# VinAIResearch/GeoFormer

Hardware: AMD Instinct MI355X
Metric: scenes/sec forward (ScanNetV2 ~150k pts) (higher is better)
Workload: dtype f32

## Files before the change

### geoformer_amd/csrc/host_draw.hip

```cpp
#include <stdint.h>
#include <stdlib.h>
#include <string.h>

#include "common.h"

#if defined(__x86_64__) && !defined(__HIP_DEVICE_COMPILE__)
#include <immintrin.h>
#define GF_DRAW_AVX2 1
#endif

namespace {
constexpr int MT_N = 624, MT_M = 397;

__attribute__((always_inline)) inline void mt_advance_body(uint32_t* key) {
    constexpr uint32_t A = 0x9908b0dfu, UP = 0x80000000u, LO = 0x7fffffffu;
    int i = 0;
    for (; i < MT_N - MT_M; i++) {
        const uint32_t y = (key[i] & UP) | (key[i + 1] & LO);
        key[i] = key[i + MT_M] ^ (y >> 1) ^ ((0u - (y & 1u)) & A);
    }
    for (; i < MT_N - 1; i++) {
        const uint32_t y = (key[i] & UP) | (key[i + 1] & LO);
        key[i] = key[i + (MT_M - MT_N)] ^ (y >> 1) ^ ((0u - (y & 1u)) & A);
    }
// ... 257 lines not shown
    }
    if (out)
        for (long long t = 0; t < k; t++) out[t] = (long long)x[t];
    if (out32 && (uint32_t*)out32 != x) memcpy(out32, x, (size_t)k * sizeof(int32_t));
    *pos_io = pos;
    return GF_OK;
}

__global__ void k_take_drawn(const int32_t* __restrict__ idx, int k, int n, const float* __restrict__ xyz_src,
                             long long* __restrict__ idx64, float* __restrict__ xyz_dst, int32_t* __restrict__ idx32) {
    const int t = blockIdx.x * blockDim.x + threadIdx.x;
    if (t >= k) return;
    const int j = idx[t];
    idx64[t] = j;
    idx32[t] = j;
    if ((unsigned)j >= (unsigned)n) return;
    xyz_dst[3 * t + 0] = xyz_src[3 * (size_t)j + 0];
    xyz_dst[3 * t + 1] = xyz_src[3 * (size_t)j + 1];
    xyz_dst[3 * t + 2] = xyz_src[3 * (size_t)j + 2];
}

extern "C" int gf_host_draw_sample(uint32_t* key, int32_t* pos_io, long long n, long long k, int32_t* pinned,
                                   long long pinned_cap, int32_t* d_idx32, long long* d_idx64, const float* xyz_src,
                                   float* xyz_dst, int fps_m, int32_t* fps_idx, void* fps_scratch, void* stream) {
    GF_CHECK_ARG(key && pos_io && pinned && d_idx32 && d_idx64 && xyz_src && xyz_dst, "gf_host_draw_sample: null argument");
    GF_CHECK_ARG(n >= 1 && n <= 0x7fffffffLL && k >= 1 && k <= n && pinned_cap >= k, "gf_host_draw_sample: n=%lld k=%lld cap=%lld",
                 n, k, pinned_cap);
    GF_CHECK_ARG(*pos_io >= 0 && *pos_io <= MT_N, "gf_host_draw_sample: generator position %d", (int)*pos_io);
    const int rc = legacy_choice32(key, pos_io, n, k, pinned, pinned_cap);
    if (rc != GF_OK) return rc;
    hipStream_t st = (hipStream_t)stream;
    hipLaunchKernelGGL(k_take_drawn, dim3((unsigned)gf_div_up(k, 256)), dim3(256), 0, st, pinned, (int)k, (int)n, xyz_src, d_idx64,
                       xyz_dst, d_idx32);
    GF_CHECK_LAUNCH("gf_host_draw_sample");
    if (fps_m > 0) {
        GF_CHECK_ARG(fps_idx && fps_scratch, "gf_host_draw_sample: sampling outputs missing");
        return gf_furthest_point_sampling(xyz_dst, 1, (int)k, fps_m, fps_idx, fps_scratch, stream);
    }
    return GF_OK;
}
```

### geoformer_amd/csrc/pointops.hip

```cpp
#include <stdlib.h>

#include <type_traits>

#include "common.h"

__global__ void k_voxelize_fp(const float* __restrict__ feats, const int32_t* __restrict__ rules, int M, int maxActive,
                              int C, int average, float* __restrict__ out) {
    long long t = (long long)blockIdx.x * blockDim.x + threadIdx.x;
    if (t >= (long long)M * C) return;
    const int row = (int)(t / C), c = (int)(t - (long long)row * C);
    const int32_t* r = rules + (size_t)row * (maxActive + 1);
    const int n = r[0];
    const float mult = (average && n > 0) ? __fdiv_rn(1.0f, (float)n) : 1.0f;
    float acc = 0.f;
    for (int i = 1; i <= n; i++) acc = __fadd_rn(acc, __fmul_rn(mult, feats[(size_t)r[i] * C + c]));
    out[t] = acc;
}

__global__ void k_voxelize_bp(const float* __restrict__ d_out, const int32_t* __restrict__ rules, int M, int maxActive,
                              int C, int average, float* __restrict__ d_feats) {
    long long t = (long long)blockIdx.x * blockDim.x + threadIdx.x;
    if (t >= (long long)M * C) return;
    const int row = (int)(t / C), c = (int)(t - (long long)row * C);
    const int32_t* r = rules + (size_t)row * (maxActive + 1);
// ... 249 lines not shown
    if (__popcll(owners) == 1) {
        key = (unsigned)__builtin_amdgcn_readlane((int)key, __builtin_ctzll(owners));
    } else {
        const unsigned cand = dbits == md ? (FPS_KEY_NONE - key) : 0u;
        key = FPS_KEY_NONE - wave_max_u32(cand);
    }
    dbits = md;
}

template <int I, int N, typename F>
__device__ __forceinline__ void fps_static_for(F&& f) {
    if constexpr (I < N) {
        f(std::integral_constant<int, I>{});
        fps_static_for<I + 1, N>(f);
    }
}

#ifndef FPS_WAVES
#define FPS_WAVES 16
#endif
#ifndef FPS_MAXG
#define FPS_MAXG 16
#endif
#ifndef FPS_KPUB
#define FPS_KPUB 4
#endif
#ifndef FPS_K
#define FPS_K 16
#endif
#define FPS_PW (FPS_WAVES - FPS_WAVES / 4)
#ifndef FPS_POLL_SLEEP
#define FPS_POLL_SLEEP 4
#endif
#define FPS_NG (FPS_MAXG * FPS_KPUB / 64)
#define FPS_TAG (1ull << 63)

__device__ __forceinline__ unsigned long long fps_code(unsigned dbits, unsigned key) {
    return ((unsigned long long)dbits << 32) | ((unsigned long long)(FPS_KEY_NONE - key) << 1);
}
__device__ __forceinline__ unsigned long long wave_max_u64(unsigned long long c) {
    const unsigned hi = (unsigned)(c >> 32), md = wave_max_u32(hi);
    const unsigned long long owners = __ballot(hi == md);
    unsigned ml;
    if (__popcll(owners) == 1) {
        ml = (unsigned)__builtin_amdgcn_readlane((int)(unsigned)c, __builtin_ctzll(owners));
    } else {
        ml = wave_max_u32(hi == md ? (unsigned)c : 0u);
    }
    return ((unsigned long long)md << 32) | ml;
}
__device__ __forceinline__ int fps_code_index(unsigned long long c) {
    return c ? (int)((FPS_KEY_NONE - (unsigned)((c >> 1) & 0x7fffffffull)) & 0x3fffffu) : 0;
}

#ifdef FPS_TRACE
__device__ unsigned long long* g_fps_trace = nullptr;
extern "C" int gf_dev_fps_trace(void* p) {
// ... 4 lines not shown
#define FTA(i, a, b) do { ftr[i] += (b) - (a); } while (0)
#else
#define FT() 0ull
#define FTA(i, a, b) do { } while (0)
#endif

#define FPS_LDS_ST(p, v) __hip_atomic_store((p), (v), __ATOMIC_RELAXED, __HIP_MEMORY_SCOPE_WORKGROUP)
#define FPS_LDS_LD(p) __hip_atomic_load((p), __ATOMIC_RELAXED, __HIP_MEMORY_SCOPE_WORKGROUP)
#define FPS_ORDER() asm volatile("" ::: "memory")
template <int P>
__device__ __forceinline__ void fps_absorb(const float (&px)[P], const float (&py)[P], const float (&pz)[P], float (&tmp)[P],
                                           float ax, float ay, float az) {
#pragma unroll
    for (int i = 0; i < P; i++) {
        const float dx = px[i] - ax, dy = py[i] - ay, dz = pz[i] - az;
        tmp[i] = fminf(fmaf(dz, dz, fmaf(dy, dy, dx * dx)), tmp[i]);
    }
}

template <int P>
__global__ __launch_bounds__(FPS_WAVES * 64) void k_fps(const float* __restrict__ xyz, int n, int m, int m0, int G,
                                                        int bs_log2, int batch0,
                                                        unsigned long long* __restrict__ slots,
                                                        int32_t* __restrict__ idxs, int* __restrict__ err) {
    static_assert(FPS_NG >= 1 && FPS_NG * 64 == FPS_MAXG * FPS_KPUB && FPS_KPUB <= FPS_K && FPS_WAVES * 2 <= 64,
                  "lane mappings of the exchange");
    __shared__ unsigned long long s_part[2][FPS_WAVES * 2];
    __shared__ float s_xyz[2][FPS_K * 3];
    __shared__ unsigned s_prog[2];
    const int bi = batch0 + blockIdx.y, wg = blockIdx.x;
    xyz += (size_t)bi * n * 3;
    idxs += (size_t)bi * m;
    slots += (size_t)bi * 2 * FPS_MAXG * FPS_KPUB;
    const int lane = threadIdx.x & 63, wid = threadIdx.x >> 6;
    const bool holder = (wid & 3) != 0;
    const int hid = wid - 1 - (wid >> 2);
    const int gtid = (wg * FPS_PW + hid) * 64 + lane;
    const int stride = G * FPS_PW * 64;
    if (threadIdx.x < 2) s_prog[threadIdx.x] = 0u;
    if (!holder && lane < 4) s_part[lane >> 1][wid * 2 + (lane & 1)] = 0ull;

    float px[P], py[P], pz[P], tmp[P];
    unsigned key[P];
    unsigned elig = 0;
    const unsigned bs_mask = (1u << bs_log2) - 1u;
#pragma unroll
    for (int i = 0; i < P; i++) {
        const int k = gtid + i * stride;
        px[i] = py[i] = pz[i] = 0.f;
        tmp[i] = 1e10f;
        key[i] = FPS_KEY_NONE;
        if (holder && k < n) {
            px[i] = xyz[(size_t)k * 3 + 0];
            py[i] = xyz[(size_t)k * 3 + 1];
            pz[i] = xyz[(size_t)k * 3 + 2];
            const float mag = fmaf(pz[i], pz[i], fmaf(py[i], py[i], px[i] * px[i]));
            if (!((double)mag <= 1e-3)) elig |= 1u << i;
            const unsigned rev = bs_log2 ? (__brev((unsigned)k & bs_mask) >> (32 - bs_log2)) : 0u;
            key[i] = (rev << 22) | (unsigned)k;
        }
    }
    if (m0 <= 0 && wg == 0 && threadIdx.x == 0) idxs[0] = 0;
    int nnew = 1;
    float nx[FPS_K], ny[FPS_K], nz[FPS_K];
    nx[0] = xyz[0]; ny[0] = xyz[1]; nz[0] = xyz[2];
#pragma unroll
    for (int a = 1; a < FPS_K; a++) nx[a] = ny[a] = nz[a] = 0.f;
    int done = 1;
    if (m0 > 1) {
        for (int base = 0; base < m0 - 1; base += FPS_K) {
            const int cntk = min(FPS_K, m0 - 1 - base);
#pragma unroll
            for (int a = 0; a < FPS_K; a++) {
                const int pi = a < cntk ? idxs[base + a] : 0;
                nx[a] = xyz[(size_t)pi * 3 + 0];
                ny[a] = xyz[(size_t)pi * 3 + 1];
                nz[a] = xyz[(size_t)pi * 3 + 2];
            }
#pragma unroll
            for (int i = 0; i < P; i++) {
                if (elig & (1u << i)) {
                    float d2 = tmp[i];
#pragma unroll
                    for (int a = 0; a < FPS_K; a++) {
                        if (a < cntk) {
                            const float dx = px[i] - nx[a], dy = py[i] - ny[a], dz = pz[i] - nz[a];
                            d2 = fminf(fmaf(dz, dz, fmaf(dy, dy, dx * dx)), d2);
                        }
                    }
                    tmp[i] = d2;
                }
            }
        }
        const int pl = idxs[m0 - 1];
        nx[0] = xyz[(size_t)pl * 3 + 0];
        ny[0] = xyz[(size_t)pl * 3 + 1];
        nz[0] = xyz[(size_t)pl * 3 + 2];
        done = m0;
    }
#ifdef FPS_TRACE
    unsigned long long ftr[10] = {0, 0, 0, 0, 0, 0, 0, 0, 0, 0};
#endif
    if (holder) {
#pragma unroll
        for (int i = 0; i < P; i++) {
            if (elig & (1u << i)) {
                const float dx = px[i] - nx[0], dy = py[i] - ny[0], dz = pz[i] - nz[0];
// ... 2 lines not shown
        }
    } else {
        __builtin_amdgcn_s_setprio(3);
    }
    __syncthreads();
    for (int round = 1; done < m; round++) {
        const int par = round & 1;
        const unsigned long long ft0 = FT();
        unsigned bd = 0u, bk = FPS_KEY_NONE;
#pragma unroll
        for (int i = 0; i < P; i++) {
            if (elig & (1u << i)) {
                float d2 = tmp[i];
                const unsigned db = __float_as_uint(d2);
                if (db > bd || (db == bd && key[i] < bk)) {
                    bd = db;
                    bk = key[i];
                }
            }
        }
        const unsigned long long ft1 = FT();
        FTA(0, ft0, ft1);
        if (holder) {
        unsigned d1 = bd, k1 = bk;
        wave_best(d1, k1);
        unsigned cd = bd, ck = bk;
        if (bk == k1 && k1 != FPS_KEY_NONE) {
            cd = 0u;
            ck = FPS_KEY_NONE;
#pragma unroll
            for (int i = 0; i < P; i++) {
                if ((elig & (1u << i)) && key[i] != k1) {
                    const unsigned db = __float_as_uint(tmp[i]);
                    if (db > cd || (db == cd && key[i] < ck)) {
                        cd = db;
                        ck = key[i];
                    }
                }
            }
        }
        unsigned d2w = cd, k2w = ck;
        wave_best(d2w, k2w);
        if (lane == 0) {
            unsigned long long c1 = fps_code(d1, k1), c2 = fps_code(d2w, k2w);
            if (c2 != 0ull) c2 |= 1ull;
            else if (c1 != 0ull) c1 |= 1ull;
            s_part[par][wid * 2 + 0] = c1;
            s_part[par][wid * 2 + 1] = c2;
        }
        }
        const unsigned long long ft2 = FT();
        FTA(1, ft1, ft2);
        __syncthreads();
        const unsigned long long ft3 = FT();
        FTA(2, ft2, ft3);
        if (wid == 0) {
            unsigned long long mine = lane < FPS_WAVES * 2 ? s_part[par][lane] : 0ull;
            unsigned long long wgc[FPS_KPUB];
            bool stop = false;
            int cnt = 0;
            fps_static_for<0, FPS_KPUB>([&](auto tc) {
                constexpr int t = decltype(tc)::value;
                const unsigned long long best = stop ? 0ull : wave_max_u64(mine);
                wgc[t] = best & ~1ull;
                if (best != 0ull) {
                    if (mine == best) mine = 0ull;
                    if (best & 1ull) stop = true;
                    cnt = t + 1;
                } else {
                    stop = true;
                }
            });
#pragma unroll
            for (int t = 0; t < FPS_KPUB; t++)
                if (t == cnt - 1) wgc[t] |= 1ull;
            const unsigned long long ft4 = FT();
            FTA(3, ft3, ft4);
            unsigned long long v[FPS_NG];
            v[0] = wgc[0];
#pragma unroll
// ... 16 lines not shown
                    v[j] = 0ull;
                }
                int spins = 0;
                while (!all) {
                    all = true;
#pragma unroll
                    for (int j = 0; j < FPS_NG; j++) {
                        if (!ok[j]) {
                            v[j] = __hip_atomic_load(rs + lane + 64 * j, __ATOMIC_RELAXED, __HIP_MEMORY_SCOPE_AGENT);
                            ok[j] = (v[j] & FPS_TAG) == tag;
                            all = all && ok[j];
                        }
                    }
                    if (++spins > FPS_SPIN_LIMIT) {
                        *err = 1;
                        break;
                    }
                }
#pragma unroll
                for (int j = 0; j < FPS_NG; j++) v[j] = (lane + 64 * j < G * FPS_KPUB) ? (v[j] & ~FPS_TAG) : 0ull;
            }
            const unsigned long long ft5 = FT();
            FTA(4, ft4, ft5);
            float vx[FPS_NG], vy[FPS_NG], vz[FPS_NG];
#pragma unroll
            for (int j = 0; j < FPS_NG; j++) {
                const int ci = fps_code_index(v[j]);
                vx[j] = xyz[(size_t)ci * 3 + 0];
                vy[j] = xyz[(size_t)ci * 3 + 1];
                vz[j] = xyz[(size_t)ci * 3 + 2];
            }
            static_assert(FPS_NG == 1, "one gathered candidate per lane");
#ifdef FPS_TRACE
            {
                float probe = vx[0];
                asm volatile("v_mov_b32 %0, %0" : "+v"(probe));
                vx[0] = probe;
            }
#endif
            const unsigned long long ft6 = FT();
            FTA(5, ft5, ft6);
            const unsigned long long mine0 = v[0];
            const unsigned long long Bcode = wave_max_u64((mine0 & 1ull) ? (mine0 & ~1ull) : 0ull);
            unsigned ckey = (unsigned)((mine0 >> 1) & 0x7fffffffull);
            float cdist = __uint_as_float((unsigned)(mine0 >> 32));
            bool alive = mine0 != 0ull;
            int nacc = 0;
            float kx = 0.f, ky = 0.f, kz = 0.f;
            int kidx = 0;
            bool direct = false;
            const unsigned clo = ckey << 1;
            const unsigned Bhi = (unsigned)(Bcode >> 32), Blo = (unsigned)Bcode;
            auto take = [&](int ol, unsigned best_lo, int t) {
                const float bx = __int_as_float(__builtin_amdgcn_readlane(__float_as_int(vx[0]), ol));
                const float by = __int_as_float(__builtin_amdgcn_readlane(__float_as_int(vy[0]), ol));
                const float bz = __int_as_float(__builtin_amdgcn_readlane(__float_as_int(vz[0]), ol));
                const bool keeper = lane == t;
                kx = keeper ? bx : kx;
                ky = keeper ? by : ky;
                kz = keeper ? bz : kz;
                kidx = keeper ? (int)((FPS_KEY_NONE - ((best_lo >> 1) & 0x7fffffffu)) & 0x3fffffu) : kidx;
                if (lane == ol) alive = false;
                if (lane == 0) {
                    FPS_LDS_ST(&s_xyz[par][t * 3 + 0], bx);
                    FPS_LDS_ST(&s_xyz[par][t * 3 + 1], by);
                    FPS_LDS_ST(&s_xyz[par][t * 3 + 2], bz);
// ... 66 lines not shown
                __builtin_amdgcn_s_sleep(FPS_POLL_SLEEP);
            }
            nnew = seen;
        } else {
            const unsigned tag = (unsigned)round << 8;
            unsigned c;
            for (;;) {
                c = FPS_LDS_LD(&s_prog[par]);
                if ((c & 0xffffff80u) == (tag | 0x80u)) break;
                __builtin_amdgcn_s_sleep(32);
            }
            nnew = (int)(c & 0x7fu);
        }
        done += nnew;
#ifdef FPS_TRACE
        ftr[8] += 1;
        ftr[9] += nnew;
#endif
    }
#ifdef FPS_TRACE
    if (g_fps_trace && wg == 0 && threadIdx.x == 0)
        for (int i = 0; i < 10; i++) g_fps_trace[i] = ftr[i];
#endif
}

template <int P>
static void launch_fps(int G, int nb, hipStream_t st, const float* xyz, int n, int m, int m0, int bs_log2, int batch0,
                       unsigned long long* slots, int32_t* idxs, int* err) {
    GF_LAUNCH_OP(GF_OP_FPS, (k_fps<P>), dim3(G, nb), dim3(FPS_WAVES * 64), 0, st, xyz, n, m, m0, G, bs_log2, batch0, slots,
                 idxs, err);
}

extern "C" size_t gf_fps_scratch_bytes(int b) {
    return ((size_t)b * 2 * FPS_MAXG * FPS_KPUB + 8) * sizeof(unsigned long long);
}

extern "C" int gf_furthest_point_sampling_resume(const float* xyz, int b, int n, int m, int m_known, int32_t* idxs,
                                                 void* scratch, void* stream);

extern "C" int gf_furthest_point_sampling(const float* xyz, int b, int n, int m, int32_t* idxs, void* scratch,
                                          void* stream) {
    return gf_furthest_point_sampling_resume(xyz, b, n, m, 0, idxs, scratch, stream);
}

extern "C" int gf_furthest_point_sampling_resume(const float* xyz, int b, int n, int m, int m_known, int32_t* idxs,
                                                 void* scratch, void* stream) {
    GF_CHECK_ARG(b >= 0 && n >= 1 && m >= 0, "gf_furthest_point_sampling: bad sizes b=%d n=%d m=%d", b, n, m);
    GF_CHECK_ARG(m_known >= 0 && m_known <= m, "gf_furthest_point_sampling_resume: m_known=%d not in [0, m=%d]", m_known,
                 m);
    if (m_known == m && m > 0) return GF_OK;
    GF_CHECK_ARG(n < (1 << 22), "gf_furthest_point_sampling: n=%d exceeds the 22-bit index of the tie-break key", n);
    if (b == 0 || m == 0) return GF_OK;
    hipStream_t st = (hipStream_t)stream;
    int bs_log2 = 0;
    while ((2 << bs_log2) <= n && bs_log2 < 9) bs_log2++;
    const int per_wg = FPS_PW * 64;
    int G = (2 * n + per_wg * 5 - 1) / (per_wg * 5);
    if (G < 1) G = 1;
    if (G > FPS_MAXG) G = FPS_MAXG;
    const int P = (n + G * per_wg - 1) / (G * per_wg);
    GF_CHECK_ARG(P <= 22, "gf_furthest_point_sampling: n=%d too large (max %d)", n, FPS_MAXG * per_wg * 22);
    unsigned long long* slots = (unsigned long long*)scratch;
    int* err = (int*)(slots + (size_t)b * 2 * FPS_MAXG * FPS_KPUB);
    GF_TRY(hipMemsetAsync(scratch, 0, gf_fps_scratch_bytes(b), st));
    const int per_launch = 1024 / (G * FPS_WAVES) > 0 ? 1024 / (G * FPS_WAVES) : 1;
    for (int b0 = 0; b0 < b; b0 += per_launch) {
        const int nb = (b - b0) < per_launch ? (b - b0) : per_launch;
        if (P <= 1) launch_fps<1>(G, nb, st, xyz, n, m, m_known, bs_log2, b0, slots, idxs, err);
        else if (P <= 2) launch_fps<2>(G, nb, st, xyz, n, m, m_known, bs_log2, b0, slots, idxs, err);
        else if (P <= 3) launch_fps<3>(G, nb, st, xyz, n, m, m_known, bs_log2, b0, slots, idxs, err);
        else if (P <= 4) launch_fps<4>(G, nb, st, xyz, n, m, m_known, bs_log2, b0, slots, idxs, err);
        else if (P <= 5) launch_fps<5>(G, nb, st, xyz, n, m, m_known, bs_log2, b0, slots, idxs, err);
        else if (P <= 6) launch_fps<6>(G, nb, st, xyz, n, m, m_known, bs_log2, b0, slots, idxs, err);
        else if (P <= 8) launch_fps<8>(G, nb, st, xyz, n, m, m_known, bs_log2, b0, slots, idxs, err);
        else if (P <= 12) launch_fps<12>(G, nb, st, xyz, n, m, m_known, bs_log2, b0, slots, idxs, err);
        else if (P <= 16) launch_fps<16>(G, nb, st, xyz, n, m, m_known, bs_log2, b0, slots, idxs, err);
        else if (P <= 20) launch_fps<20>(G, nb, st, xyz, n, m, m_known, bs_log2, b0, slots, idxs, err);
        else launch_fps<22>(G, nb, st, xyz, n, m, m_known, bs_log2, b0, slots, idxs, err);
    }
    GF_CHECK_LAUNCH("gf_furthest_point_sampling");
    return GF_OK;
}
```

### geoformer_amd/model/geoformer.py

```python
from __future__ import annotations

import functools
import os

import numpy as np
import torch
import torch.nn as nn
from torch.nn import functional as F

from .. import _lib, pointops, spconv, unet_exec, unet_train
from . import config as _config
from .backbone import ResidualBlock, UBlock, conv1d_bn_relu, random_downsample
from .layers import (BatchNorm1d, BigLinear, GenericMLP, LazyRelPos, PointwiseConv1d, PositionEmbeddingCoordsSine, RelPosSpec,
                     TransformerDecoder,
                     TransformerDecoderLayer, scene_counts)
from .set_abstraction import PointnetSAModuleVotesSeparate


class _Voxelization(torch.autograd.Function):

    @staticmethod
    def forward(ctx, feats, map_rule, mode=4):
        ctx.rule, ctx.mode, ctx.N = map_rule, mode, feats.shape[0]
        return pointops.voxelize_fp(feats.contiguous(), map_rule, mode)
# ... 491 lines not shown
            for b in range(batch_size):
                n_b = offs[b + 1] - offs[b]
                if n_b == 0:
                    return None
                npoint = min(n_b, self.cfg.n_downsampling)
                draw = pointops.legacy_choice(n_b, npoint) if locs_float_.is_cuda else \
                    np.random.choice(n_b, npoint, replace=False)
                sampling_indices = torch.tensor(draw, dtype=torch.long, device=locs_float_.device)
                self.last_sampling_indices = sampling_indices
                xyz_b = locs_float_[offs[b]:offs[b + 1]][sampling_indices].unsqueeze(0)
                feat_b = output_feats_[offs[b]:offs[b + 1]][sampling_indices].unsqueeze(0)
                l, gf, gx, idx = self.set_aggregator.group_points(xyz_b.contiguous(),
                                                                  feat_b.transpose(1, 2).contiguous())
                locs.append(l); gfeat.append(gf); gxyz.append(gx); inds.append(idx)
            context_locs, pre_enc_inds = torch.cat(locs), torch.cat(inds)
            context_feats = self.set_aggregator.mlp(torch.cat(gfeat), torch.cat(gxyz)).transpose(1, 2)
            return context_locs, context_feats, pre_enc_inds

    def _sampling_split(self):
        nq = self.cfg.n_query_points
        npoint_sa = self.set_aggregator.npoint
        return nq, npoint_sa, os.environ.get("GF_OVERLAP", "1") != "2" and npoint_sa > nq

    def _first_picks(self, xyz_b, sb, first=None, xyz_ready=None):
        nq, npoint_sa, split = self._sampling_split()
        if xyz_ready is None:
            xyz_ready = torch.cuda.Event()
            xyz_ready.record(sb)
        if first is None:
            first = pointops.furthest_point_sampling(xyz_b, nq if split else npoint_sa)
        src = first[0, :nq].contiguous()
        first_ready = torch.cuda.Event()
        first_ready.record(sb)
        idx = pointops.furthest_point_sampling(xyz_b, npoint_sa, known=first) if split else first
        fps_done = torch.cuda.Event()
        fps_done.record(sb)
        return xyz_ready, first, src, first_ready, idx, fps_done

    def _sample_from_count(self, n, locs_rows, bufs):
        npoint = min(n, self.cfg.n_downsampling)
        drawn = pointops.draw_sample(n, npoint, locs_rows, bufs)
        if drawn is None:
            return None
        sampling_indices, xyz_b = drawn[:2]
        sb = torch.cuda.current_stream()
        if len(drawn) == 3:
            first_ready = torch.cuda.Event()
            first_ready.record(sb)
            return (sampling_indices, xyz_b) + self._first_picks(xyz_b, sb, first=drawn[2], xyz_ready=first_ready)
        return (sampling_indices, xyz_b) + self._first_picks(xyz_b, sb)

    def _aggregate_geodesic_overlapped(self, locs_float_, output_feats_, batch_offsets_, batch_size, graphs, max_step,
                                       pc_dims=None, sample=True, epilogue=True, early=None, presampled=None,
                                       presampled_before=None):
        offs = _offsets_list(batch_offsets_)
        grad_ctx = self._grad_ctx("set_aggregator")
        nq, npoint_sa, split = self._sampling_split()
        main = torch.cuda.current_stream()
        sides = _SIDE_STREAMS
        side = sides.get((locs_float_.device, main.cuda_stream))
        if side is None:
            side = torch.cuda.Stream(device=locs_float_.device)
            sides[(locs_float_.device, main.cuda_stream)] = side
        aux = sides.get((locs_float_.device, main.cuda_stream, "aux"))
        if aux is None:
            aux = sides[(locs_float_.device, main.cuda_stream, "aux")] = torch.cuda.Stream(device=locs_float_.device)
        geo_ready = [None] * batch_size
        staged, geo = [None] * batch_size, [None] * batch_size
        fps_done_evs = []
        multi = batch_size > 1 and early is None and not epilogue
        scene_streams = []
        def host_draw(b, n_b):
# ... 655 lines not shown
```

### geoformer_amd/pointops.py

```python
from __future__ import annotations

import contextlib
import os
import threading

import numpy as np
import torch

from . import _lib
from ._lib import check, ptr, stream_ptr


def _f32c(t, name):
    if not (t.is_cuda and t.dtype == torch.float32 and t.is_contiguous()):
        raise RuntimeError(f"{name}: expected a contiguous float32 tensor on the GPU")
    return t


def _i32c(t, name):
    if not (t.is_cuda and t.dtype == torch.int32 and t.is_contiguous()):
        raise RuntimeError(f"{name}: expected a contiguous int32 tensor on the GPU")
    return t


# ... 72 lines not shown
    check(_lib.load().gf_group_points_grad(ptr(grad_out), ptr(idx), b, c, n, npoints, nsample, ptr(out),
                                           stream_ptr()), "gf_group_points_grad")
    return out


def ball_query(new_xyz, xyz, radius, nsample, grid=None):
    _f32c(new_xyz, "new_xyz"); _f32c(xyz, "xyz")
    b, m, _ = new_xyz.shape
    n = xyz.shape[1]
    idx = torch.empty((b, m, nsample), dtype=torch.int32, device=xyz.device)
    lib = _lib.load()
    if grid is None:
        grid = b == 1 and n >= 4096
    if grid and b == 1 and n >= 1:
        scratch = torch.empty(lib.gf_knn_scratch_bytes(n) // 4 + 16, dtype=torch.int32, device=xyz.device)
        check(lib.gf_ball_query_grid(ptr(xyz), n, None, ptr(new_xyz), m, float(radius), nsample, ptr(scratch), 0, None,
                                     ptr(idx), stream_ptr()), "gf_ball_query_grid")
        return idx
    check(lib.gf_ball_query(ptr(new_xyz), ptr(xyz), b, n, m, float(radius), nsample, ptr(idx), stream_ptr()),
          "gf_ball_query")
    return idx


def furthest_point_sampling(xyz, m, known=None):
    _f32c(xyz, "xyz")
    b, n, _ = xyz.shape
    lib = _lib.load()
    idx = torch.empty((b, m), dtype=torch.int32, device=xyz.device)
    scratch = torch.empty(lib.gf_fps_scratch_bytes(b) // 8 + 1, dtype=torch.int64, device=xyz.device)
    m0 = 0
    if known is not None:
        _i32c(known, "known")
        m0 = min(int(known.shape[1]), m)
        idx[:, :m0] = known[:, :m0]
    check(lib.gf_furthest_point_sampling_resume(ptr(xyz), b, n, m, m0, ptr(idx), ptr(scratch), stream_ptr()),
          "gf_furthest_point_sampling")
    return idx


def select_foreground(scores, cls, equal, locs, batch_idxs, feats, feat_rows=None, deferred=False):
    _f32c(scores, "scores"); _f32c(locs, "locs"); _i32c(batch_idxs, "batch_idxs"); _f32c(feats, "feats")
    if feat_rows is not None:
        _i32c(feat_rows, "feat_rows")
    N, C = scores.shape
    F = feats.shape[1]
    dev = scores.device
    lib = _lib.load()
    scratch = torch.empty(lib.gf_fg_scratch_bytes(N) // 4 + 1, dtype=torch.int32, device=dev)
    fg = torch.empty(N, dtype=torch.int64, device=dev)
    locs_o = torch.empty((N, 3), dtype=torch.float32, device=dev)
    bidx_o = torch.empty(N, dtype=torch.int32, device=dev)
    feats_o = torch.empty((N, F), dtype=torch.float32, device=dev)
    scores_o = torch.empty((N, C), dtype=torch.float32, device=dev)
    cnt = torch.empty(1, dtype=torch.int32, device=dev)
    host = PendingForeground.take_word() if deferred else None
    check(lib.gf_fg_select(ptr(scores), N, C, int(cls), int(bool(equal)), ptr(locs), ptr(batch_idxs), ptr(feats),
                           ptr(feat_rows), F,
                           ptr(scratch), ptr(fg), ptr(locs_o), ptr(bidx_o), ptr(feats_o), ptr(scores_o), ptr(cnt),
# ... 95 lines not shown
        return
    st = np.random.get_state()
    if st[0] != "MT19937":
        return
    key = np.ascontiguousarray(st[1], dtype=np.uint32)
    check(_lib.load().gf_host_legacy_prefetch(key.ctypes.data, int(st[2]), int(nwords)), "gf_host_legacy_prefetch")


_DRAW_PINS = {}


def draw_sample_buffers(kmax, n_cap, device, fps_m=0):
    key = (device.index, stream_ptr())
    pin = _DRAW_PINS.get(key)
    if pin is None or pin.numel() < max(n_cap, kmax):
        pin = _DRAW_PINS[key] = torch.empty(max(n_cap + n_cap // 4, kmax, 65536), dtype=torch.int32).pin_memory()
    bufs = {"pin": pin, "idx32": torch.empty(kmax, dtype=torch.int32, device=device),
            "idx64": torch.empty(kmax, dtype=torch.int64, device=device),
            "xyz": torch.empty((1, kmax, 3), dtype=torch.float32, device=device), "kmax": kmax, "fps_m": 0}
    if fps_m > 0:
        bufs["fps_m"] = int(fps_m)
        bufs["fps_idx"] = torch.empty((1, int(fps_m)), dtype=torch.int32, device=device)
        bufs["fps_scratch"] = torch.empty(_lib.load().gf_fps_scratch_bytes(1) // 8 + 1, dtype=torch.int64, device=device)
    return bufs


def draw_sample(n, k, xyz_src, bufs):
    n, k = int(n), int(k)
    direct = _legacy_state() if 1 <= k <= n <= 0x7fffffff and k <= bufs["kmax"] else None
    if direct is None:
        return None
    _f32c(xyz_src, "xyz_src")
    addr, lock = direct
    pin = bufs["pin"]
    fps_m = bufs["fps_m"] if 0 < bufs["fps_m"] <= k else 0
    with lock:
        check(_lib.load().gf_host_draw_sample(addr, addr + 2496, n, k, pin.data_ptr(), pin.numel(), ptr(bufs["idx32"]),
                                              ptr(bufs["idx64"]), ptr(xyz_src), ptr(bufs["xyz"]), fps_m,
                                              ptr(bufs["fps_idx"]) if fps_m else None,
                                              ptr(bufs["fps_scratch"]) if fps_m else None, stream_ptr()),
              "gf_host_draw_sample")
    if fps_m:
        return bufs["idx64"][:k], bufs["xyz"][:, :k], bufs["fps_idx"]
    return bufs["idx64"][:k], bufs["xyz"][:, :k]


def legacy_choice(n, k, out=None):
    import ctypes

    import numpy as np

    n, k = int(n), int(k)
    direct = _legacy_state() if 1 <= k <= n <= 0x7fffffff else None
    if direct is not None:
        addr, lock = direct
        if out is None or out.dtype != np.int64 or out.size < k or not out.flags.c_contiguous:
            out = np.empty(k, dtype=np.int64)
        with lock:
            check(_lib.load().gf_host_legacy_choice(addr, addr + 2496, n, k, out.ctypes.data), "gf_host_legacy_choice")
        return out[:k]
    st = np.random.get_state()
    if st[0] != "MT19937" or not (1 <= k <= n <= 0x7fffffff):
        return np.random.choice(n, k, replace=False)
# ... 1236 lines not shown
```

### include/geoformer_hip.h

```cpp
#ifndef GEOFORMER_HIP_H
#define GEOFORMER_HIP_H

#include <stddef.h>
#include <stdint.h>

#ifdef __cplusplus
extern "C" {
#endif

#define GF_ABI_VERSION 7

typedef enum {
    GF_OK = 0,
    GF_ERR_INVALID_ARG = -1,
    GF_ERR_LAUNCH = -2,
    GF_ERR_UNSUPPORTED = -3,
    GF_ERR_CALLBACK = -4,
} gf_status;

int gf_abi_version(void);
const char* gf_last_error(void);

size_t gf_fg_scratch_bytes(int N);
int gf_fg_select(const float* scores, int N, int C, int cls, int mode, const float* locs, const int32_t* batch_idxs,
                 const float* feats, const int32_t* feat_rows, int F, void* scratch, long long* fg_idxs, float* locs_out,
                 int32_t* bidx_out, float* feats_out, float* scores_out, int32_t* d_count, int32_t* h_count, void* stream);
int gf_host_wait_word(const volatile int32_t* word, int pending, long long timeout_us);

int gf_host_legacy_choice(uint32_t* key, int32_t* pos, long long n, long long k, long long* out);
int gf_host_legacy_prefetch(const uint32_t* key, int pos, long long nwords);
int gf_host_draw_sample(uint32_t* key, int32_t* pos, long long n, long long k, int32_t* pinned, long long pinned_cap,
                        int32_t* d_idx32, long long* d_idx64, const float* xyz_src, float* xyz_dst, int fps_m,
                        int32_t* fps_idx, void* fps_scratch, void* stream);


size_t gf_index_words(int B, int X, int Y, int Z);
size_t gf_index_scratch_bytes(size_t words);

int gf_index_build(const int32_t* coords, int M, const int32_t* d_M, int B, int X, int Y, int Z, uint32_t* bitmap,
                   int32_t* prefix, int32_t* perm, void* scratch, void* stream);

size_t gf_rules_steps_words(int ld);
int gf_rules_subm3(const int32_t* coords, int M, const int32_t* d_M, int X, int Y, int Z, const uint32_t* bitmap,
                   const int32_t* prefix, const int32_t* perm, int32_t* nbr, int ld, uint32_t* gmask, int32_t* steps,
                   void* stream);

int gf_rules_down2(const int32_t* coords, int M, const int32_t* d_M, int B, int X, int Y, int Z,
                   uint32_t* bitmap_out, int32_t* prefix_out, void* scratch, int32_t* out_coords,
                   int32_t* d_M_out, int32_t* child, int ld, int32_t* parent, int32_t* koff, int32_t* up, int ld_up,
                   uint32_t* gmask_down, uint32_t* gmask_up, void* stream);

int gf_rules_down2_chain_plan(int M0, int B, int X, int Y, int Z, int nlevels, long long* offsets, int* caps, int* shapes,
                              long long* ws_elems, int* nlevels_out);
int gf_rules_down2_chain(const int32_t* coords, int M0, int B, int X, int Y, int Z, int nlevels, int32_t* ws,
                         int32_t* counts, void* stream);

// ... 145 lines not shown
int gf_feeder_wait_copied(void* feeder, int slot);
int gf_feeder_wait_head(void* feeder, int slot);
int gf_feeder_destroy(void* feeder);

int gf_voxelize_fp(const float* feats, const int32_t* rules, int M, int maxActive, int C, int average, float* out,
                   void* stream);
int gf_voxelize_bp(const float* d_out, const int32_t* rules, int M, int maxActive, int C, int average, float* d_feats,
                   void* stream);


int gf_gather_points(const float* points, const int32_t* idx, int b, int c, int n, int m, float* out, void* stream);
int gf_gather_points_grad(const float* grad_out, const int32_t* idx, int b, int c, int n, int m, float* grad_points,
                          void* stream);
int gf_group_points(const float* points, const int32_t* idx, int b, int c, int n, int npoints, int nsample, float* out,
                    void* stream);
int gf_group_points_grad(const float* grad_out, const int32_t* idx, int b, int c, int n, int npoints, int nsample,
                         float* grad_points, void* stream);
int gf_ball_query(const float* new_xyz, const float* xyz, int b, int n, int m, float radius, int nsample, int32_t* idx,
                  void* stream);
size_t gf_fps_scratch_bytes(int b);
int gf_furthest_point_sampling(const float* xyz, int b, int n, int m, int32_t* idxs, void* scratch, void* stream);
int gf_furthest_point_sampling_resume(const float* xyz, int b, int n, int m, int m_known, int32_t* idxs,
                                      void* scratch, void* stream);


size_t gf_knn_scratch_bytes(int n);
int gf_knn_radius(const float* xyz, int n, int k, float radius, int sqrt_out, float* D, int32_t* I, int32_t* deg,
                  void* scratch, void* stream);
const int32_t* gf_knn_error_flag(void* scratch, int n);

size_t gf_geodesic_bfs_queue_words(int n);
int gf_geodesic_bfs(const float* D, const int32_t* I, const int32_t* deg, int n, int K, const int32_t* src, int nq,
                    float radius, int max_step, float* geo, void* keys_ws, void* queue_ws, void* stream);
int gf_geodesic_bfs_cfg(const float* D, const int32_t* I, const int32_t* deg, int n, int K, const int32_t* src, int nq,
                        float radius, int max_step, float* geo, void* keys_ws, void* queue_ws, size_t queue_words,
                        int wg_threads, void* stream);

int gf_mask_head(const float* feat, const float* coords, const float* geo, const float* qxyz,
                 const float* sqrt_max_geo, const float* w1, const float* b1, const float* w2, const float* b2, int N,
                 int nq, int C, float* out, void* stream);
int gf_mask_head_packed(const float* feat, const float* coords, const float* geo, const float* qxyz,
                        const float* sqrt_max_geo, const float* w1, const float* b1, const float* w2, const float* b2,
                        int ldp, int N, int nq, int C, float* out, void* stream);
size_t gf_mask_head_split_bytes(int N);
int gf_mask_head_episodes(const float* feat, const float* coords, const float* geo, const float* qxyz,
                          const float* sqrt_max_geo, const float* w1, const float* b1, const float* w2, const float* b2,
// ... 275 lines not shown
```

Measured before the change: 227.6.

## Persist FPS min-distance state across split launches and widen per-wave candidate exchange

When furthest point sampling runs in two phases (first nq picks, then resume to the full count), the first launch now saves each point's running min distance into a state buffer with a validity header. The resume launch reloads that state instead of recomputing distances to all known picks. Separately, each wave now publishes its top three candidates instead of two, and each workgroup publishes eight instead of four, with a DPP-based merge, so fewer rounds need a full exchange. This adds a state buffer of size n per batch, extra stores and header checks, and more exchange traffic per round.

Measured after the change: 228.0 (median of 2 runs). Within noise of the previous version (+0.2%).

```diff
diff --git a/geoformer_amd/csrc/host_draw.hip b/geoformer_amd/csrc/host_draw.hip
--- a/geoformer_amd/csrc/host_draw.hip
+++ b/geoformer_amd/csrc/host_draw.hip
@@ -303,7 +303,8 @@
 
 extern "C" int gf_host_draw_sample(uint32_t* key, int32_t* pos_io, long long n, long long k, int32_t* pinned,
                                    long long pinned_cap, int32_t* d_idx32, long long* d_idx64, const float* xyz_src,
-                                   float* xyz_dst, int fps_m, int32_t* fps_idx, void* fps_scratch, void* stream) {
+                                   float* xyz_dst, int fps_m, int32_t* fps_idx, void* fps_scratch, void* fps_state,
+                                   void* stream) {
     GF_CHECK_ARG(key && pos_io && pinned && d_idx32 && d_idx64 && xyz_src && xyz_dst, "gf_host_draw_sample: null argument");
     GF_CHECK_ARG(n >= 1 && n <= 0x7fffffffLL && k >= 1 && k <= n && pinned_cap >= k, "gf_host_draw_sample: n=%lld k=%lld cap=%lld",
                  n, k, pinned_cap);
@@ -316,7 +317,7 @@
     GF_CHECK_LAUNCH("gf_host_draw_sample");
     if (fps_m > 0) {
         GF_CHECK_ARG(fps_idx && fps_scratch, "gf_host_draw_sample: sampling outputs missing");
-        return gf_furthest_point_sampling(xyz_dst, 1, (int)k, fps_m, fps_idx, fps_scratch, stream);
+        return gf_furthest_point_sampling_state(xyz_dst, 1, (int)k, fps_m, 0, fps_idx, fps_scratch, fps_state, stream);
     }
     return GF_OK;
 }
diff --git a/geoformer_amd/csrc/pointops.hip b/geoformer_amd/csrc/pointops.hip
--- a/geoformer_amd/csrc/pointops.hip
+++ b/geoformer_amd/csrc/pointops.hip
@@ -295,17 +295,24 @@
 #ifndef FPS_MAXG
 #define FPS_MAXG 16
 #endif
+#ifndef FPS_WTOP
+#define FPS_WTOP 3
+#endif
 #ifndef FPS_KPUB
-#define FPS_KPUB 4
+#define FPS_KPUB 8
 #endif
 #ifndef FPS_K
-#define FPS_K 16
-#endif
+#define FPS_K 24
+#endif
+#define FPS_RK 16
 #define FPS_PW (FPS_WAVES - FPS_WAVES / 4)
 #ifndef FPS_POLL_SLEEP
 #define FPS_POLL_SLEEP 4
 #endif
 #define FPS_NG (FPS_MAXG * FPS_KPUB / 64)
+#define FPS_STATE_HDR 32
+#define FPS_STATE_GEN 0x46505331u
+#define FPS_STATE_WORDS(n) ((size_t)FPS_STATE_HDR + (((size_t)(n) + 31) & ~(size_t)31))
 #define FPS_TAG (1ull << 63)
 
 __device__ __forceinline__ unsigned long long fps_code(unsigned dbits, unsigned key) {
@@ -356,14 +363,17 @@
 __global__ __launch_bounds__(FPS_WAVES * 64) void k_fps(const float* __restrict__ xyz, int n, int m, int m0, int G,
                                                         int bs_log2, int batch0,
                                                         unsigned long long* __restrict__ slots,
-                                                        int32_t* __restrict__ idxs, int* __restrict__ err) {
-    static_assert(FPS_NG >= 1 && FPS_NG * 64 == FPS_MAXG * FPS_KPUB && FPS_KPUB <= FPS_K && FPS_WAVES * 2 <= 64,
+                                                        int32_t* __restrict__ idxs, int* __restrict__ err,
+                                                        unsigned* __restrict__ state, int state_mode) {
+    static_assert(FPS_NG >= 1 && FPS_NG <= 2 && FPS_NG * 64 == FPS_MAXG * FPS_KPUB && FPS_KPUB <= FPS_K &&
+                      (FPS_KPUB & (FPS_KPUB - 1)) == 0 && FPS_K <= 64 && FPS_WTOP >= 1 && FPS_WAVES * FPS_WTOP <= 64,
                   "lane mappings of the exchange");
-    __shared__ unsigned long long s_part[2][FPS_WAVES * 2];
+    __shared__ unsigned long long s_part[2][FPS_WAVES * FPS_WTOP];
     __shared__ float s_xyz[2][FPS_K * 3];
     __shared__ unsigned s_prog[2];
     const int bi = batch0 + blockIdx.y, wg = blockIdx.x;
     xyz += (size_t)bi * n * 3;
+    if (state_mode) state += (size_t)bi * FPS_STATE_WORDS(n);
     idxs += (size_t)bi * m;
     slots += (size_t)bi * 2 * FPS_MAXG * FPS_KPUB;
     const int lane = threadIdx.x & 63, wid = threadIdx.x >> 6;
@@ -372,7 +382,8 @@
     const int gtid = (wg * FPS_PW + hid) * 64 + lane;
     const int stride = G * FPS_PW * 64;
     if (threadIdx.x < 2) s_prog[threadIdx.x] = 0u;
-    if (!holder && lane < 4) s_part[lane >> 1][wid * 2 + (lane & 1)] = 0ull;
+    if (!holder && lane < 2 * FPS_WTOP)
+        s_part[lane / FPS_WTOP][wid * FPS_WTOP + lane % FPS_WTOP] = 0ull;
 
     float px[P], py[P], pz[P], tmp[P];
     unsigned key[P];
@@ -395,17 +406,41 @@
         }
     }
     if (m0 <= 0 && wg == 0 && threadIdx.x == 0) idxs[0] = 0;
+    if (state_mode == 1 && wg == 0 && threadIdx.x == 0) {
+        const unsigned long long xa = (unsigned long long)(uintptr_t)xyz;
+        state[1] = (unsigned)n;
+        state[2] = (unsigned)m;
+        state[3] = (unsigned)G;
+        state[4] = (unsigned)P;
+        state[6] = (unsigned)xa;
+        state[7] = (unsigned)(xa >> 32);
+    }
     int nnew = 1;
-    float nx[FPS_K], ny[FPS_K], nz[FPS_K];
+    float nx[FPS_RK], ny[FPS_RK], nz[FPS_RK];
     nx[0] = xyz[0]; ny[0] = xyz[1]; nz[0] = xyz[2];
 #pragma unroll
-    for (int a = 1; a < FPS_K; a++) nx[a] = ny[a] = nz[a] = 0.f;
+    for (int a = 1; a < FPS_RK; a++) nx[a] = ny[a] = nz[a] = 0.f;
     int done = 1;
     if (m0 > 1) {
-        for (int base = 0; base < m0 - 1; base += FPS_K) {
-            const int cntk = min(FPS_K, m0 - 1 - base);
-#pragma unroll
-            for (int a = 0; a < FPS_K; a++) {
+        bool loaded = false;
+        if (state_mode == 2) {
+            const unsigned long long xa = (unsigned long long)(uintptr_t)xyz;
+            loaded = state[1] == (unsigned)n && state[2] == (unsigned)m0 && state[3] == (unsigned)G &&
+                     state[4] == (unsigned)P && state[5] == (unsigned)idxs[m0 - 1] && state[6] == (unsigned)xa &&
+                     state[7] == (unsigned)(xa >> 32);
+#pragma unroll
+            for (int g = 0; g < FPS_MAXG; g++) loaded = loaded && (g >= G || state[16 + g] == FPS_STATE_GEN);
+            if (loaded && holder) {
+                const float* sd = (const float*)(state + FPS_STATE_HDR);
+#pragma unroll
+                for (int i = 0; i < P; i++)
+                    if (gtid + i * stride < n) tmp[i] = sd[(size_t)i * stride + gtid];
+            }
+        }
+        for (int base = 0; !loaded && base < m0 - 1; base += FPS_RK) {
+            const int cntk = min(FPS_RK, m0 - 1 - base);
+#pragma unroll
+            for (int a = 0; a < FPS_RK; a++) {
                 const int pi = a < cntk ? idxs[base + a] : 0;
                 nx[a] = xyz[(size_t)pi * 3 + 0];
                 ny[a] = xyz[(size_t)pi * 3 + 1];
@@ -416,7 +451,7 @@
                 if (elig & (1u << i)) {
                     float d2 = tmp[i];
 #pragma unroll
-                    for (int a = 0; a < FPS_K; a++) {
+                    for (int a = 0; a < FPS_RK; a++) {
                         if (a < cntk) {
                             const float dx = px[i] - nx[a], dy = py[i] - ny[a], dz = pz[i] - nz[a];
                             d2 = fminf(fmaf(dz, dz, fmaf(dy, dy, dx * dx)), d2);
@@ -465,32 +500,45 @@
         const unsigned long long ft1 = FT();
         FTA(0, ft0, ft1);
         if (holder) {
-        unsigned d1 = bd, k1 = bk;
-        wave_best(d1, k1);
-        unsigned cd = bd, ck = bk;
-        if (bk == k1 && k1 != FPS_KEY_NONE) {
-            cd = 0u;
-            ck = FPS_KEY_NONE;
-#pragma unroll
-            for (int i = 0; i < P; i++) {
-                if ((elig & (1u << i)) && key[i] != k1) {
-                    const unsigned db = __float_as_uint(tmp[i]);
-                    if (db > cd || (db == cd && key[i] < ck)) {
-                        cd = db;
-                        ck = key[i];
+            unsigned long long wc[FPS_WTOP];
+            unsigned wk[FPS_WTOP];
+            fps_static_for<0, FPS_WTOP>([&](auto tc) {
+                constexpr int t = decltype(tc)::value;
+                unsigned d1 = bd, k1 = bk;
+                wave_best(d1, k1);
+                wc[t] = fps_code(d1, k1);
+                wk[t] = k1;
+                if constexpr (t + 1 < FPS_WTOP) {
+                    if (bk == k1 && k1 != FPS_KEY_NONE) {
+                        bd = 0u;
+                        bk = FPS_KEY_NONE;
+#pragma unroll
+                        for (int i = 0; i < P; i++) {
+                            bool fresh = (elig & (1u << i)) != 0u;
+#pragma unroll
+                            for (int u = 0; u <= t; u++) fresh = fresh && key[i] != wk[u];
+                            if (fresh) {
+                                const unsigned db = __float_as_uint(tmp[i]);
+                                if (db > bd || (db == bd && key[i] < bk)) {
+                                    bd = db;
+                                    bk = key[i];
+                                }
+                            }
+                        }
                     }
                 }
-            }
-        }
-        unsigned d2w = cd, k2w = ck;
-        wave_best(d2w, k2w);
-        if (lane == 0) {
-            unsigned long long c1 = fps_code(d1, k1), c2 = fps_code(d2w, k2w);
-            if (c2 != 0ull) c2 |= 1ull;
-            else if (c1 != 0ull) c1 |= 1ull;
-            s_part[par][wid * 2 + 0] = c1;
-            s_part[par][wid * 2 + 1] = c2;
-        }
+            });
+            if (lane == 0) {
+                bool flagged = false;
+#pragma unroll
+                for (int t = FPS_WTOP - 1; t >= 0; t--) {
+                    if (!flagged && wc[t] != 0ull) {
+                        wc[t] |= 1ull;
+                        flagged = true;
+                    }
+                    s_part[par][wid * FPS_WTOP + t] = wc[t];
+                }
+            }
         }
         const unsigned long long ft2 = FT();
         FTA(1, ft1, ft2);
@@ -498,7 +546,7 @@
         const unsigned long long ft3 = FT();
         FTA(2, ft2, ft3);
         if (wid == 0) {
-            unsigned long long mine = lane < FPS_WAVES * 2 ? s_part[par][lane] : 0ull;
+            unsigned long long mine = lane < FPS_WAVES * FPS_WTOP ? s_part[par][lane] : 0ull;
             unsigned long long wgc[FPS_KPUB];
             bool stop = false;
             int cnt = 0;
@@ -561,15 +609,25 @@
             }
             const unsigned long long ft5 = FT();
             FTA(4, ft4, ft5);
-            float vx[FPS_NG], vy[FPS_NG], vz[FPS_NG];
-#pragma unroll
-            for (int j = 0; j < FPS_NG; j++) {
-                const int ci = fps_code_index(v[j]);
-                vx[j] = xyz[(size_t)ci * 3 + 0];
-                vy[j] = xyz[(size_t)ci * 3 + 1];
-                vz[j] = xyz[(size_t)ci * 3 + 2];
-            }
-            static_assert(FPS_NG == 1, "one gathered candidate per lane");
+            static_assert(FPS_NG == 1 || FPS_KPUB == 8, "row_half_mirror pairs the ranks of a prefix of 8");
+            unsigned long long dropped = 0ull;
+#pragma unroll
+            for (int j = 1; j < FPS_NG; j++) {
+                const unsigned mlo = (unsigned)__builtin_amdgcn_update_dpp(0, (int)(unsigned)v[j], 0x141, 0xF, 0xF, true);
+                const unsigned mhi = (unsigned)__builtin_amdgcn_update_dpp(0, (int)(unsigned)(v[j] >> 32), 0x141, 0xF, 0xF, true);
+                v[j] = ((unsigned long long)mhi << 32) | mlo;
+                const unsigned long long lo = v[j] < v[0] ? v[j] : v[0];
+                v[0] = v[j] < v[0] ? v[0] : v[j];
+                dropped = lo > dropped ? lo : dropped;
+            }
+            dropped &= ~1ull;
+            float vx[1], vy[1], vz[1];
+            {
+                const int ci = fps_code_index(v[0]);
+                vx[0] = xyz[(size_t)ci * 3 + 0];
+                vy[0] = xyz[(size_t)ci * 3 + 1];
+                vz[0] = xyz[(size_t)ci * 3 + 2];
+            }
 #ifdef FPS_TRACE
             {
                 float probe = vx[0];
@@ -580,7 +638,8 @@
             const unsigned long long ft6 = FT();
             FTA(5, ft5, ft6);
             const unsigned long long mine0 = v[0];
-            const unsigned long long Bcode = wave_max_u64((mine0 & 1ull) ? (mine0 & ~1ull) : 0ull);
+            const unsigned long long Bown = (mine0 & 1ull) ? (mine0 & ~1ull) : 0ull;
+            const unsigned long long Bcode = wave_max_u64(Bown > dropped ? Bown : dropped);
             unsigned ckey = (unsigned)((mine0 >> 1) & 0x7fffffffull);
             float cdist = __uint_as_float((unsigned)(mine0 >> 32));
             bool alive = mine0 != 0ull;
@@ -693,29 +752,52 @@
     if (g_fps_trace && wg == 0 && threadIdx.x == 0)
         for (int i = 0; i < 10; i++) g_fps_trace[i] = ftr[i];
 #endif
+    if (state_mode == 1) {
+        if (holder) {
+            const int k0 = (blockIdx.x * FPS_PW + hid) * 64 + __lane_id();
+            float* sd = (float*)(state + FPS_STATE_HDR);
+#pragma unroll
+            for (int i = 0; i < P; i++) {
+                const int k = k0 + i * (G * FPS_PW * 64);
+                if (k < n) sd[k] = tmp[i];
+            }
+        }
+        __threadfence();
+        __syncthreads();
+        if (threadIdx.x == 0) {
+            if (blockIdx.x == 0) state[5] = (unsigned)idxs[m - 1];
+            __hip_atomic_store(state + 16 + blockIdx.x, FPS_STATE_GEN, __ATOMIC_RELEASE, __HIP_MEMORY_SCOPE_AGENT);
+        }
+    }
 }
 
 template <int P>
 static void launch_fps(int G, int nb, hipStream_t st, const float* xyz, int n, int m, int m0, int bs_log2, int batch0,
-                       unsigned long long* slots, int32_t* idxs, int* err) {
+                       unsigned long long* slots, int32_t* idxs, int* err, unsigned* state, int state_mode) {
     GF_LAUNCH_OP(GF_OP_FPS, (k_fps<P>), dim3(G, nb), dim3(FPS_WAVES * 64), 0, st, xyz, n, m, m0, G, bs_log2, batch0, slots,
-                 idxs, err);
+                 idxs, err, state, state_mode);
 }
 
 extern "C" size_t gf_fps_scratch_bytes(int b) {
     return ((size_t)b * 2 * FPS_MAXG * FPS_KPUB + 8) * sizeof(unsigned long long);
 }
 
-extern "C" int gf_furthest_point_sampling_resume(const float* xyz, int b, int n, int m, int m_known, int32_t* idxs,
-                                                 void* scratch, void* stream);
+extern "C" size_t gf_fps_state_bytes(int b, int n) {
+    return (size_t)(b > 0 ? b : 0) * FPS_STATE_WORDS(n > 0 ? n : 0) * sizeof(unsigned);
+}
 
 extern "C" int gf_furthest_point_sampling(const float* xyz, int b, int n, int m, int32_t* idxs, void* scratch,
                                           void* stream) {
-    return gf_furthest_point_sampling_resume(xyz, b, n, m, 0, idxs, scratch, stream);
+    return gf_furthest_point_sampling_state(xyz, b, n, m, 0, idxs, scratch, nullptr, stream);
 }
 
 extern "C" int gf_furthest_point_sampling_resume(const float* xyz, int b, int n, int m, int m_known, int32_t* idxs,
                                                  void* scratch, void* stream) {
+    return gf_furthest_point_sampling_state(xyz, b, n, m, m_known, idxs, scratch, nullptr, stream);
+}
+
+extern "C" int gf_furthest_point_sampling_state(const float* xyz, int b, int n, int m, int m_known, int32_t* idxs,
+                                                void* scratch, void* state, void* stream) {
     GF_CHECK_ARG(b >= 0 && n >= 1 && m >= 0, "gf_furthest_point_sampling: bad sizes b=%d n=%d m=%d", b, n, m);
     GF_CHECK_ARG(m_known >= 0 && m_known <= m, "gf_furthest_point_sampling_resume: m_known=%d not in [0, m=%d]", m_known,
                  m);
@@ -734,20 +816,24 @@
     unsigned long long* slots = (unsigned long long*)scratch;
     int* err = (int*)(slots + (size_t)b * 2 * FPS_MAXG * FPS_KPUB);
     GF_TRY(hipMemsetAsync(scratch, 0, gf_fps_scratch_bytes(b), st));
+    const int state_mode = !state ? 0 : m_known > 1 ? 2 : m_known == 0 ? 1 : 0;
+    if (state_mode == 1)
+        GF_TRY(hipMemset2DAsync(state, FPS_STATE_WORDS(n) * sizeof(unsigned), 0, FPS_STATE_HDR * sizeof(unsigned), (size_t)b,
+                                st));
     const int per_launch = 1024 / (G * FPS_WAVES) > 0 ? 1024 / (G * FPS_WAVES) : 1;
     for (int b0 = 0; b0 < b; b0 += per_launch) {
         const int nb = (b - b0) < per_launch ? (b - b0) : per_launch;
-        if (P <= 1) launch_fps<1>(G, nb, st, xyz, n, m, m_known, bs_log2, b0, slots, idxs, err);
-        else if (P <= 2) launch_fps<2>(G, nb, st, xyz, n, m, m_known, bs_log2, b0, slots, idxs, err);
-        else if (P <= 3) launch_fps<3>(G, nb, st, xyz, n, m, m_known, bs_log2, b0, slots, idxs, err);
-        else if (P <= 4) launch_fps<4>(G, nb, st, xyz, n, m, m_known, bs_log2, b0, slots, idxs, err);
-        else if (P <= 5) launch_fps<5>(G, nb, st, xyz, n, m, m_known, bs_log2, b0, slots, idxs, err);
-        else if (P <= 6) launch_fps<6>(G, nb, st, xyz, n, m, m_known, bs_log2, b0, slots, idxs, err);
-        else if (P <= 8) launch_fps<8>(G, nb, st, xyz, n, m, m_known, bs_log2, b0, slots, idxs, err);
-        else if (P <= 12) launch_fps<12>(G, nb, st, xyz, n, m, m_known, bs_log2, b0, slots, idxs, err);
-        else if (P <= 16) launch_fps<16>(G, nb, st, xyz, n, m, m_known, bs_log2, b0, slots, idxs, err);
-        else if (P <= 20) launch_fps<20>(G, nb, st, xyz, n, m, m_known, bs_log2, b0, slots, idxs, err);
-        else launch_fps<22>(G, nb, st, xyz, n, m, m_known, bs_log2, b0, slots, idxs, err);
+        if (P <= 1) launch_fps<1>(G, nb, st, xyz, n, m, m_known, bs_log2, b0, slots, idxs, err, (unsigned*)state, state_mode);
+        else if (P <= 2) launch_fps<2>(G, nb, st, xyz, n, m, m_known, bs_log2, b0, slots, idxs, err, (unsigned*)state, state_mode);
+        else if (P <= 3) launch_fps<3>(G, nb, st, xyz, n, m, m_known, bs_log2, b0, slots, idxs, err, (unsigned*)state, state_mode);
+        else if (P <= 4) launch_fps<4>(G, nb, st, xyz, n, m, m_known, bs_log2, b0, slots, idxs, err, (unsigned*)state, state_mode);
+        else if (P <= 5) launch_fps<5>(G, nb, st, xyz, n, m, m_known, bs_log2, b0, slots, idxs, err, (unsigned*)state, state_mode);
+        else if (P <= 6) launch_fps<6>(G, nb, st, xyz, n, m, m_known, bs_log2, b0, slots, idxs, err, (unsigned*)state, state_mode);
+        else if (P <= 8) launch_fps<8>(G, nb, st, xyz, n, m, m_known, bs_log2, b0, slots, idxs, err, (unsigned*)state, state_mode);
+        else if (P <= 12) launch_fps<12>(G, nb, st, xyz, n, m, m_known, bs_log2, b0, slots, idxs, err, (unsigned*)state, state_mode);
+        else if (P <= 16) launch_fps<16>(G, nb, st, xyz, n, m, m_known, bs_log2, b0, slots, idxs, err, (unsigned*)state, state_mode);
+        else if (P <= 20) launch_fps<20>(G, nb, st, xyz, n, m, m_known, bs_log2, b0, slots, idxs, err, (unsigned*)state, state_mode);
+        else launch_fps<22>(G, nb, st, xyz, n, m, m_known, bs_log2, b0, slots, idxs, err, (unsigned*)state, state_mode);
     }
     GF_CHECK_LAUNCH("gf_furthest_point_sampling");
     return GF_OK;
diff --git a/geoformer_amd/model/geoformer.py b/geoformer_amd/model/geoformer.py
--- a/geoformer_amd/model/geoformer.py
+++ b/geoformer_amd/model/geoformer.py
@@ -537,17 +537,18 @@
         npoint_sa = self.set_aggregator.npoint
         return nq, npoint_sa, os.environ.get("GF_OVERLAP", "1") != "2" and npoint_sa > nq
 
-    def _first_picks(self, xyz_b, sb, first=None, xyz_ready=None):
+    def _first_picks(self, xyz_b, sb, first=None, xyz_ready=None, state=None):
         nq, npoint_sa, split = self._sampling_split()
         if xyz_ready is None:
             xyz_ready = torch.cuda.Event()
             xyz_ready.record(sb)
         if first is None:
-            first = pointops.furthest_point_sampling(xyz_b, nq if split else npoint_sa)
+            state = pointops.fps_state(xyz_b.shape[0], xyz_b.shape[1], xyz_b.device) if split else None
+            first = pointops.furthest_point_sampling(xyz_b, nq if split else npoint_sa, state=state)
         src = first[0, :nq].contiguous()
         first_ready = torch.cuda.Event()
         first_ready.record(sb)
-        idx = pointops.furthest_point_sampling(xyz_b, npoint_sa, known=first) if split else first
+        idx = pointops.furthest_point_sampling(xyz_b, npoint_sa, known=first, state=state) if split else first
         fps_done = torch.cuda.Event()
         fps_done.record(sb)
         return xyz_ready, first, src, first_ready, idx, fps_done
@@ -562,7 +563,8 @@
         if len(drawn) == 3:
             first_ready = torch.cuda.Event()
             first_ready.record(sb)
-            return (sampling_indices, xyz_b) + self._first_picks(xyz_b, sb, first=drawn[2], xyz_ready=first_ready)
+            return (sampling_indices, xyz_b) + self._first_picks(xyz_b, sb, first=drawn[2], xyz_ready=first_ready,
+                                                                 state=bufs.get("fps_state"))
         return (sampling_indices, xyz_b) + self._first_picks(xyz_b, sb)
 
     def _aggregate_geodesic_overlapped(self, locs_float_, output_feats_, batch_offsets_, batch_size, graphs, max_step,
diff --git a/geoformer_amd/pointops.py b/geoformer_amd/pointops.py
--- a/geoformer_amd/pointops.py
+++ b/geoformer_amd/pointops.py
@@ -118,7 +118,11 @@
     return idx
 
 
-def furthest_point_sampling(xyz, m, known=None):
+def fps_state(b, n, device):
+    return torch.empty(_lib.load().gf_fps_state_bytes(int(b), int(n)) // 4, dtype=torch.int32, device=device)
+
+
+def furthest_point_sampling(xyz, m, known=None, state=None):
     _f32c(xyz, "xyz")
     b, n, _ = xyz.shape
     lib = _lib.load()
@@ -129,7 +133,12 @@
         _i32c(known, "known")
         m0 = min(int(known.shape[1]), m)
         idx[:, :m0] = known[:, :m0]
-    check(lib.gf_furthest_point_sampling_resume(ptr(xyz), b, n, m, m0, ptr(idx), ptr(scratch), stream_ptr()),
+    if state is not None:
+        _i32c(state, "state")
+        if state.numel() * 4 < lib.gf_fps_state_bytes(b, n):
+            raise ValueError("furthest_point_sampling: state buffer too small for b=%d n=%d" % (b, n))
+    check(lib.gf_furthest_point_sampling_state(ptr(xyz), b, n, m, m0, ptr(idx), ptr(scratch),
+                                               ptr(state) if state is not None else None, stream_ptr()),
           "gf_furthest_point_sampling")
     return idx
 
@@ -271,6 +280,7 @@
         bufs["fps_m"] = int(fps_m)
         bufs["fps_idx"] = torch.empty((1, int(fps_m)), dtype=torch.int32, device=device)
         bufs["fps_scratch"] = torch.empty(_lib.load().gf_fps_scratch_bytes(1) // 8 + 1, dtype=torch.int64, device=device)
+        bufs["fps_state"] = fps_state(1, kmax, device)
     return bufs
 
 
@@ -287,7 +297,8 @@
         check(_lib.load().gf_host_draw_sample(addr, addr + 2496, n, k, pin.data_ptr(), pin.numel(), ptr(bufs["idx32"]),
                                               ptr(bufs["idx64"]), ptr(xyz_src), ptr(bufs["xyz"]), fps_m,
                                               ptr(bufs["fps_idx"]) if fps_m else None,
-                                              ptr(bufs["fps_scratch"]) if fps_m else None, stream_ptr()),
+                                              ptr(bufs["fps_scratch"]) if fps_m else None,
+                                              ptr(bufs["fps_state"]) if fps_m else None, stream_ptr()),
               "gf_host_draw_sample")
     if fps_m:
         return bufs["idx64"][:k], bufs["xyz"][:, :k], bufs["fps_idx"]
diff --git a/include/geoformer_hip.h b/include/geoformer_hip.h
--- a/include/geoformer_hip.h
+++ b/include/geoformer_hip.h
@@ -31,7 +31,7 @@
 int gf_host_legacy_prefetch(const uint32_t* key, int pos, long long nwords);
 int gf_host_draw_sample(uint32_t* key, int32_t* pos, long long n, long long k, int32_t* pinned, long long pinned_cap,
                         int32_t* d_idx32, long long* d_idx64, const float* xyz_src, float* xyz_dst, int fps_m,
-                        int32_t* fps_idx, void* fps_scratch, void* stream);
+                        int32_t* fps_idx, void* fps_scratch, void* fps_state, void* stream);
 
 
 size_t gf_index_words(int B, int X, int Y, int Z);
@@ -223,6 +223,9 @@
 int gf_furthest_point_sampling(const float* xyz, int b, int n, int m, int32_t* idxs, void* scratch, void* stream);
 int gf_furthest_point_sampling_resume(const float* xyz, int b, int n, int m, int m_known, int32_t* idxs,
                                       void* scratch, void* stream);
+size_t gf_fps_state_bytes(int b, int n);
+int gf_furthest_point_sampling_state(const float* xyz, int b, int n, int m, int m_known, int32_t* idxs, void* scratch,
+                                     void* state, void* stream);
 
 
 size_t gf_knn_scratch_bytes(int n);
```
